# microsoft/UniVL

Measured on NVIDIA H100. Metric: video-text samples/sec, higher is better.
Workload: dtype bf16

## Files before the change

univl_b200/csrc/common.cuh:

```cuda
#pragma once

#include <cuda.h>
#include <cuda_bf16.h>
#include <cuda_runtime.h>
#include <stdint.h>
#include <stdio.h>

namespace univl {

typedef __nv_bfloat16 bf16;

int set_error(int code, const char* fmt, ...);
int device_sms();
int usable_sms();
int scratch_alloc(void** p, size_t bytes, cudaStream_t st);
int partials_reduce(float* part, int nparts, long long rows, long long cols, float* dst, long long ld, cudaStream_t st);
#define UNIVL_OK 0
#define UNIVL_ERR_ARG -1
#define UNIVL_ERR_CUDA -2
#define UNIVL_ERR_UNSUPPORTED -3

#define UNIVL_CHECK_ARG(cond, ...)                                   \
  do {                                                               \
    if (!(cond)) return univl::set_error(UNIVL_ERR_ARG, __VA_ARGS__); \
  } while (0)

#define UNIVL_CHECK_LAUNCH(name)                                                          \
  do {                                                                                    \
    cudaError_t e__ = cudaGetLastError();                                                 \
    if (e__ != cudaSuccess)                                                               \
      return univl::set_error(UNIVL_ERR_CUDA, "%s launch: %s", name, cudaGetErrorString(e__)); \
  } while (0)

bool pdl_enabled();
__device__ __forceinline__ void pdl_trigger() { asm volatile("griddepcontrol.launch_dependents;" ::: "memory"); }
__device__ __forceinline__ void pdl_wait() { asm volatile("griddepcontrol.wait;" ::: "memory"); }

template <typename... KArgs, typename... Args>
static inline cudaError_t launch_kernel(void (*kern)(KArgs...), dim3 grid, dim3 block, size_t smem, cudaStream_t st,
                                        Args... args) {
  cudaLaunchConfig_t cfg = {};
  cfg.gridDim = grid;
  cfg.blockDim = block;
  cfg.dynamicSmemBytes = smem;
  cfg.stream = st;
  cudaLaunchAttribute attr[1];
  int n = 0;
  if (pdl_enabled()) {
    attr[n].id = cudaLaunchAttributeProgrammaticStreamSerialization;
    attr[n].val.programmaticStreamSerializationAllowed = 1;
    ++n;
  }
  cfg.attrs = attr;
  cfg.numAttrs = n;
  return cudaLaunchKernelEx(&cfg, kern, KArgs(args)...);
}

__device__ __forceinline__ uint32_t smem_u32(const void* p) {
  return static_cast<uint32_t>(__cvta_generic_to_shared(p));
}
__device__ __forceinline__ uint32_t lane_id() { return threadIdx.x & 31u; }

__device__ __forceinline__ void pair_sources(long long p, int groups, long long n_seq, long long Nb, long long& i,
                                             long long& j) {
  if (groups == 0) {
    i = j = p;
    return;
  }
  const long long Gv = Nb / groups;
  const long long g = groups > 1 ? p / (n_seq / groups) : 0;
  const long long r = p - g * (n_seq / groups);
  i = g * (n_seq / Nb) + r / Gv;
  j = g * Gv + r % Gv;
}
__device__ __forceinline__ long long pair_sequence(int which, long long owner, int f, int groups, long long Gt,
                                                   long long Gv) {
  if (groups == 0) return owner;
  if (which == 0) return owner * Gv + f;
  const long long g = owner / Gv;
  return (g * Gt + f) * Gv + (owner - g * Gv);
}

__device__ __forceinline__ float warp_sum(float v) {
#pragma unroll
  for (int o = 16; o > 0; o >>= 1) v += __shfl_xor_sync(0xffffffffu, v, o);
  return v;
}
__device__ __forceinline__ float warp_max(float v) {
#pragma unroll
  for (int o = 16; o > 0; o >>= 1) v = fmaxf(v, __shfl_xor_sync(0xffffffffu, v, o));
  return v;
}

__device__ __forceinline__ uint32_t pack_bf16x2(float lo, float hi) {
  __nv_bfloat162 v = __floats2bfloat162_rn(lo, hi);
  return *reinterpret_cast<uint32_t*>(&v);
}
__device__ __forceinline__ float2 unpack_bf16x2(uint32_t u) {
  __nv_bfloat162 v = *reinterpret_cast<__nv_bfloat162*>(&u);
  return __bfloat1622float2(v);
}

__device__ __forceinline__ float rcp_approx(float x) {
  float r;
  asm("rcp.approx.ftz.f32 %0, %1;" : "=f"(r) : "f"(x));
  return r;
}
__device__ __forceinline__ float ex2_approx(float x) {
  float r;
  asm("ex2.approx.ftz.f32 %0, %1;" : "=f"(r) : "f"(x));
  return r;
}
__device__ __forceinline__ void erf_exp_terms(float x, float& w, float& gauss) {
  const float t = rcp_approx(fmaf(fabsf(x), 0.3275911f * 0.70710678118654752440f, 1.0f));
  gauss = ex2_approx((x * x) * (-0.5f * 1.44269504088896340736f));
  float poly = fmaf(0.5f * 1.061405429f, t, 0.5f * -1.453152027f);
  poly = fmaf(poly, t, 0.5f * 1.421413741f);
  poly = fmaf(poly, t, 0.5f * -0.284496736f);
  poly = fmaf(poly, t, 0.5f * 0.254829592f);
  w = (poly * t) * gauss;
}
__device__ __forceinline__ float gelu_erf(float x) {
  float w, g;
  erf_exp_terms(x, w, g);
  return fmaf(-fabsf(x), w, fmaxf(x, 0.f));
}
__device__ __forceinline__ float gelu_erf_grad(float x) {
  float w, g;
  erf_exp_terms(x, w, g);
  const float cdf = x >= 0.f ? 1.0f - w : w;
  return fmaf(x * 0.39894228040143267794f, g, cdf);
}

__device__ __forceinline__ uint4 philox4x32(uint64_t seed, uint64_t ctr_hi, uint64_t ctr_lo) {
  uint32_t k0 = (uint32_t)seed, k1 = (uint32_t)(seed >> 32);
  uint32_t c0 = (uint32_t)ctr_lo, c1 = (uint32_t)(ctr_lo >> 32);
  uint32_t c2 = (uint32_t)ctr_hi, c3 = (uint32_t)(ctr_hi >> 32);
#pragma unroll
  for (int i = 0; i < 10; ++i) {
    const uint32_t hi0 = __umulhi(0xD2511F53u, c0), lo0 = 0xD2511F53u * c0;
    const uint32_t hi1 = __umulhi(0xCD9E8D57u, c2), lo1 = 0xCD9E8D57u * c2;
    const uint32_t n0 = hi1 ^ c1 ^ k0, n1 = lo1, n2 = hi0 ^ c3 ^ k1, n3 = lo0;
    c0 = n0; c1 = n1; c2 = n2; c3 = n3;
    k0 += 0x9E3779B9u; k1 += 0xBB67AE85u;
  }
  return make_uint4(c0, c1, c2, c3);
}

__device__ __forceinline__ bool dropout_keep(uint64_t seed, uint64_t stream, uint64_t idx,
                                             uint32_t keep_threshold) {
  const uint4 r = philox4x32(seed, stream, idx >> 2);
  const uint32_t w = (idx & 3) == 0 ? r.x : (idx & 3) == 1 ? r.y : (idx & 3) == 2 ? r.z : r.w;
  return w < keep_threshold;
}
__host__ __device__ __forceinline__ uint32_t dropout_threshold(float p) {
  double keep = 1.0 - (double)p;
  if (keep >= 1.0) return 0xFFFFFFFFu;
  return (uint32_t)(keep * 4294967296.0);
}
__host__ __device__ __forceinline__ uint32_t dropout_threshold16(float p) {
  double keep = 1.0 - (double)p;
  if (keep >= 1.0) return 65536u;
  return (uint32_t)(keep * 65536.0 + 0.5);
}
__device__ __forceinline__ uint32_t philox_u16(const uint4& r, int w) {
  const uint32_t x = (w >> 1) == 0 ? r.x : (w >> 1) == 1 ? r.y : (w >> 1) == 2 ? r.z : r.w;
  return (w & 1) ? (x >> 16) : (x & 0xFFFFu);
}
__device__ __forceinline__ uint32_t dropout_keep8(uint64_t seed, uint64_t stream, uint64_t idx0, uint32_t thr16) {
  const uint4 r = philox4x32(seed, stream, idx0 >> 3);
  return ((r.x & 0xFFFFu) < thr16 ? 1u : 0u) | ((r.x >> 16) < thr16 ? 2u : 0u) | ((r.y & 0xFFFFu) < thr16 ? 4u : 0u) |
         ((r.y >> 16) < thr16 ? 8u : 0u) | ((r.z & 0xFFFFu) < thr16 ? 16u : 0u) | ((r.z >> 16) < thr16 ? 32u : 0u) |
         ((r.w & 0xFFFFu) < thr16 ? 64u : 0u) | ((r.w >> 16) < thr16 ? 128u : 0u);
}

__device__ __forceinline__ void mbar_init(uint64_t* bar, uint32_t count) {
  asm volatile("mbarrier.init.shared::cta.b64 [%0], %1;" ::"r"(smem_u32(bar)), "r"(count) : "memory");
}
__device__ __forceinline__ void fence_mbar_init() {
  asm volatile("fence.mbarrier_init.release.cluster;" ::: "memory");
}
__device__ __forceinline__ void fence_proxy_async_smem() {
  asm volatile("fence.proxy.async.shared::cta;" ::: "memory");
}
__device__ __forceinline__ void mbar_arrive_expect_tx(uint64_t* bar, uint32_t bytes) {
  asm volatile("mbarrier.arrive.expect_tx.shared::cta.b64 _, [%0], %1;" ::"r"(smem_u32(bar)), "r"(bytes)
               : "memory");
}
__device__ __forceinline__ void mbar_arrive(uint64_t* bar) {
  asm volatile("mbarrier.arrive.shared::cta.b64 _, [%0];" ::"r"(smem_u32(bar)) : "memory");
}
__device__ __forceinline__ uint32_t mbar_try_wait(uint64_t* bar, uint32_t parity) {
  uint32_t ok;
  asm volatile(
      "{\n\t.reg .pred p;\n\t"
      "mbarrier.try_wait.parity.shared::cta.b64 p, [%1], %2;\n\t"
      "selp.b32 %0, 1, 0, p;\n\t}"
      : "=r"(ok)
      : "r"(smem_u32(bar)), "r"(parity)
      : "memory");
  return ok;
}
__device__ __forceinline__ void mbar_wait(uint64_t* bar, uint32_t parity) {
  uint32_t spins = 0;
  while (!mbar_try_wait(bar, parity)) {
    if (++spins > (1u << 26)) __trap();
  }
}

__device__ __forceinline__ void tma_prefetch_desc(const CUtensorMap* m) {
  asm volatile("prefetch.tensormap [%0];" ::"l"(reinterpret_cast<uint64_t>(m)) : "memory");
}
__device__ __forceinline__ void tma_load_2d(void* smem_dst, const CUtensorMap* m, uint64_t* bar, int c0,
                                            int c1) {
  asm volatile(
      "cp.async.bulk.tensor.2d.shared::cluster.global.tile.mbarrier::complete_tx::bytes [%0], [%1, {%2, %3}], [%4];"
      ::"r"(smem_u32(smem_dst)), "l"(reinterpret_cast<uint64_t>(m)), "r"(c0), "r"(c1), "r"(smem_u32(bar))
      : "memory");
}


__device__ __forceinline__ void tma_store_2d(const CUtensorMap* m, const void* smem_src, int c0, int c1) {
  asm volatile("cp.async.bulk.tensor.2d.global.shared::cta.tile.bulk_group [%0, {%1, %2}], [%3];" ::"l"(
                   reinterpret_cast<uint64_t>(m)),
               "r"(c0), "r"(c1), "r"(smem_u32(smem_src))
               : "memory");
}
__device__ __forceinline__ void bulk_commit() { asm volatile("cp.async.bulk.commit_group;" ::: "memory"); }
template <int N>
__device__ __forceinline__ void bulk_wait_read() {
  asm volatile("cp.async.bulk.wait_group.read %0;" ::"n"(N) : "memory");
}
__device__ __forceinline__ void bulk_wait_all() { asm volatile("cp.async.bulk.wait_group 0;" ::: "memory"); }

__device__ __forceinline__ bool elect_one() {
  uint32_t pred;
  asm volatile(
      "{\n\t.reg .pred p;\n\t"
      "elect.sync _|p, 0xffffffff;\n\t"
      "selp.b32 %0, 1, 0, p;\n\t}"
      : "=r"(pred));
  return pred != 0;
}
__device__ __forceinline__ void wgmma_fence() { asm volatile("wgmma.fence.sync.aligned;" ::: "memory"); }
__device__ __forceinline__ void wgmma_commit() { asm volatile("wgmma.commit_group.sync.aligned;" ::: "memory"); }
template <int N>
__device__ __forceinline__ void wgmma_wait() {
  asm volatile("wgmma.wait_group.sync.aligned %0;" ::"n"(N) : "memory");
}
template <int R>
__device__ __forceinline__ void fence_regs(float (&d)[R]) {
#pragma unroll
  for (int i = 0; i < R; ++i) asm volatile("" : "+f"(d[i])::"memory");
}
template <int N>
__device__ __forceinline__ void regs_dealloc() {
  asm volatile("setmaxnreg.dec.sync.aligned.u32 %0;" ::"n"(N));
}
template <int N>
__device__ __forceinline__ void regs_alloc() {
  asm volatile("setmaxnreg.inc.sync.aligned.u32 %0;" ::"n"(N));
}
__device__ __forceinline__ void named_bar(int id, int count) {
  asm volatile("bar.sync %0, %1;" ::"r"(id), "r"(count) : "memory");
}

__device__ __forceinline__ uint64_t make_smem_desc_sw128(uint32_t smem_addr, uint32_t lbo_bytes, uint32_t sbo_bytes) {
  uint64_t d = 0;
  d |= (uint64_t)((smem_addr >> 4) & 0x3FFFu);
  d |= (uint64_t)((lbo_bytes >> 4) & 0x3FFFu) << 16;
  d |= (uint64_t)((sbo_bytes >> 4) & 0x3FFFu) << 32;
  d |= (uint64_t)1 << 62;
  return d;
}

}
```

univl_b200/csrc/gemm_wgmma.cu:

```cuda
#include "common.cuh"
#include "tmap.cuh"
#include "wgmma.cuh"

#include <stdio.h>

namespace univl {

enum GemmEpilogue : int {
  EPI_BIAS_BF16 = 0,
  EPI_BIAS_GELU_BF16 = 1,
  EPI_GELU_BWD_BF16 = 2,
  EPI_ADD_BF16 = 3,
  EPI_BIAS_F32 = 4,
  EPI_ATOMIC_F32 = 5,
};

struct GemmParams {
  int M, N, Kc;
  int k_blocks_per_split;
  int epilogue;
  float alpha;
  void* out;
  long long ldo;
  const float* bias;
  const bf16* aux_in;
  long long ld_aux_in;
  bf16* aux_out;
  long long ld_aux_out;
  int vec2;
  float* part;
};

constexpr int BLOCK_M = 128;
constexpr int BLOCK_K = 64;
constexpr int GEMM_THREADS = 384;
constexpr int PLAN_SMS = 132;

template <int BLOCK_N, int STAGES>
struct GemmSmem {
  static constexpr int A_BYTES = BLOCK_M * BLOCK_K * 2;
  static constexpr int B_BYTES = BLOCK_N * BLOCK_K * 2;
  static constexpr int STAGE_BYTES = A_BYTES + B_BYTES;
  static constexpr int BAR_OFFSET = STAGES * STAGE_BYTES;
  static constexpr int TOTAL = BAR_OFFSET + 2 * STAGES * 8;
  static constexpr int DYN_BYTES = TOTAL + 1024;
  static_assert(DYN_BYTES <= 227 * 1024, "shared memory per block");
};

struct WorkItem {
  int m0, n0, kb_begin, num_kb;
};
__device__ __forceinline__ WorkItem decode_work(int w, int m_tiles, int n_tiles, int total_kb, int kb_per, int bn) {
  const int tiles = m_tiles * n_tiles;
  const int split = w / tiles;
  const int rem = w - split * tiles;
  int m_blk, n_blk;
  if (kb_per >= total_kb) {
    m_blk = rem / n_tiles;
    n_blk = rem - m_blk * n_tiles;
  } else {
    n_blk = rem / m_tiles;
    m_blk = rem - n_blk * m_tiles;
  }
  WorkItem it;
  it.m0 = m_blk * BLOCK_M;
  it.n0 = n_blk * bn;
  it.kb_begin = split * kb_per;
  it.num_kb = min(total_kb, it.kb_begin + kb_per) - it.kb_begin;
  return it;
}

__device__ __forceinline__ void epi_pair(const GemmParams& p, int split, int row, int col, float v0, float v1) {
  if (row >= p.M || col >= p.N) return;
  const bool two = col + 1 < p.N;
  const bool vec = two && p.vec2;
  const int epi = p.epilogue;
  v0 *= p.alpha;
  v1 *= p.alpha;
  if (p.bias != nullptr && (epi == EPI_BIAS_BF16 || epi == EPI_BIAS_GELU_BF16 || epi == EPI_BIAS_F32)) {
    v0 += __ldg(p.bias + col);
    if (two) v1 += __ldg(p.bias + col + 1);
  }
  if (epi == EPI_ATOMIC_F32 && p.part != nullptr) {
    float* o = p.part + ((long long)split * p.M + row) * p.N + col;
    if (two && (p.N & 1) == 0) *reinterpret_cast<float2*>(o) = make_float2(v0, v1);
    else {
      o[0] = v0;
      if (two) o[1] = v1;
    }
    return;
  }
  if (epi == EPI_ATOMIC_F32 || epi == EPI_BIAS_F32) {
    float* o = reinterpret_cast<float*>(p.out) + (long long)row * p.ldo + col;
    if (epi == EPI_ATOMIC_F32) {
      if (vec) {
        float2 a = *reinterpret_cast<float2*>(o);
        *reinterpret_cast<float2*>(o) = make_float2(a.x + v0, a.y + v1);
      } else {
        o[0] += v0;
        if (two) o[1] += v1;
      }
    } else {
      if (vec) *reinterpret_cast<float2*>(o) = make_float2(v0, v1);
      else {
        o[0] = v0;
        if (two) o[1] = v1;
      }
    }
    return;
  }
  if (epi == EPI_GELU_BWD_BF16 || epi == EPI_ADD_BF16) {
    const bf16* a = p.aux_in + (long long)row * p.ld_aux_in + col;
    float x0, x1 = 0.f;
    if (vec) {
      const float2 f = unpack_bf16x2(*reinterpret_cast<const uint32_t*>(a));
      x0 = f.x;
      x1 = f.y;
    } else {
      x0 = __bfloat162float(a[0]);
      if (two) x1 = __bfloat162float(a[1]);
    }
    if (epi == EPI_GELU_BWD_BF16) {
      v0 *= gelu_erf_grad(x0);
      v1 *= gelu_erf_grad(x1);
    } else {
      v0 += x0;
      v1 += x1;
    }
  }
  if (epi == EPI_BIAS_GELU_BF16) {
    bf16* ao = p.aux_out + (long long)row * p.ld_aux_out + col;
    if (vec) *reinterpret_cast<uint32_t*>(ao) = pack_bf16x2(v0, v1);
    else {
      ao[0] = __float2bfloat16(v0);
      if (two) ao[1] = __float2bfloat16(v1);
    }
    v0 = gelu_erf(v0);
    v1 = gelu_erf(v1);
  }
  bf16* o = reinterpret_cast<bf16*>(p.out) + (long long)row * p.ldo + col;
  if (vec) *reinterpret_cast<uint32_t*>(o) = pack_bf16x2(v0, v1);
  else {
    o[0] = __float2bfloat16(v0);
    if (two) o[1] = __float2bfloat16(v1);
  }
}

constexpr int EPI_CHUNK = 8;

template <int EPI, bool BIAS, bool PART, int BLOCK_N>
__device__ __forceinline__ void epi_tile(const GemmParams& p, int split, int row, int col0,
                                         const float (&acc)[BLOCK_N / 2]) {
  constexpr int GROUPS = BLOCK_N / 8;
  constexpr int CHUNK = GROUPS < EPI_CHUNK ? GROUPS : EPI_CHUNK;
  constexpr bool AUX = EPI == EPI_GELU_BWD_BF16 || EPI == EPI_ADD_BF16;
  constexpr bool OUT_F32 = EPI == EPI_BIAS_F32 || EPI == EPI_ATOMIC_F32;
  constexpr bool ACCUM = EPI == EPI_ATOMIC_F32 && !PART;
  const float alpha = p.alpha;
  const float* bias = p.bias + col0;
  const bf16* ax = p.aux_in + (long long)row * p.ld_aux_in + col0;
  const long long ax8 = 8 * p.ld_aux_in;
  bf16* ao = p.aux_out + (long long)row * p.ld_aux_out + col0;
  const long long ao8 = 8 * p.ld_aux_out;
  const long long ld = PART ? (long long)p.N : p.ldo;
  const long long o8 = 8 * ld;
  float* of = PART ? p.part + ((long long)split * p.M + row) * p.N + col0
                   : reinterpret_cast<float*>(p.out) + (long long)row * ld + col0;
  bf16* ob = reinterpret_cast<bf16*>(p.out) + (long long)row * ld + col0;
  float b[2][CHUNK][2];
  uint32_t x[2][CHUNK][2];
  float2 a[2][CHUNK][2];
  auto load = [&](int j0, int s) {
#pragma unroll
    for (int j = 0; j < CHUNK; ++j) {
      const int c = (j0 + j) * 8;
      if constexpr (BIAS) {
        b[s][j][0] = __ldg(bias + c);
        b[s][j][1] = __ldg(bias + c + 1);
      }
#pragma unroll
      for (int h = 0; h < 2; ++h) {
        if constexpr (AUX) x[s][j][h] = *reinterpret_cast<const uint32_t*>(ax + h * ax8 + c);
        if constexpr (ACCUM) a[s][j][h] = *reinterpret_cast<const float2*>(of + h * o8 + c);
      }
    }
  };
  load(0, 0);
#pragma unroll
  for (int j0 = 0; j0 < GROUPS; j0 += CHUNK) {
    const int s = (j0 / CHUNK) & 1;
    if (j0 + CHUNK < GROUPS) load(j0 + CHUNK, s ^ 1);
#pragma unroll
    for (int j = 0; j < CHUNK; ++j) {
      const int c = (j0 + j) * 8;
#pragma unroll
      for (int h = 0; h < 2; ++h) {
        float v0 = __fmul_rn(acc[4 * (j0 + j) + 2 * h], alpha);
        float v1 = __fmul_rn(acc[4 * (j0 + j) + 2 * h + 1], alpha);
        if constexpr (BIAS) {
          v0 = __fadd_rn(v0, b[s][j][0]);
          v1 = __fadd_rn(v1, b[s][j][1]);
        }
        if constexpr (AUX) {
          const float2 f = unpack_bf16x2(x[s][j][h]);
          if constexpr (EPI == EPI_GELU_BWD_BF16) {
            v0 = __fmul_rn(v0, gelu_erf_grad(f.x));
            v1 = __fmul_rn(v1, gelu_erf_grad(f.y));
          } else {
            v0 = __fadd_rn(v0, f.x);
            v1 = __fadd_rn(v1, f.y);
          }
        }
        if constexpr (OUT_F32) {
          if constexpr (ACCUM) {
            v0 = __fadd_rn(a[s][j][h].x, v0);
            v1 = __fadd_rn(a[s][j][h].y, v1);
          }
          *reinterpret_cast<float2*>(of + h * o8 + c) = make_float2(v0, v1);
        } else {
          if constexpr (EPI == EPI_BIAS_GELU_BF16) {
            *reinterpret_cast<uint32_t*>(ao + h * ao8 + c) = pack_bf16x2(v0, v1);
            v0 = gelu_erf(v0);
            v1 = gelu_erf(v1);
          }
          *reinterpret_cast<uint32_t*>(ob + h * o8 + c) = pack_bf16x2(v0, v1);
        }
      }
    }
  }
}

template <int BLOCK_N, int STAGES, bool A_MN, bool B_MN>
__global__ void __launch_bounds__(GEMM_THREADS, 1)
gemm_wgmma_kernel(const __grid_constant__ CUtensorMap tmap_a, const __grid_constant__ CUtensorMap tmap_b,
                  const GemmParams p, const int num_work) {
  using L = GemmSmem<BLOCK_N, STAGES>;
  pdl_trigger();
  extern __shared__ uint8_t smem_raw[];
  uint8_t* smem = reinterpret_cast<uint8_t*>((reinterpret_cast<uintptr_t>(smem_raw) + 1023) & ~uintptr_t(1023));
  uint64_t* full_bar = reinterpret_cast<uint64_t*>(smem + L::BAR_OFFSET);
  uint64_t* empty_bar = full_bar + STAGES;

  const int wg = threadIdx.x >> 7;
  const int m_tiles = (p.M + BLOCK_M - 1) / BLOCK_M;
  const int n_tiles = (p.N + BLOCK_N - 1) / BLOCK_N;
  const int total_kb = (p.Kc + BLOCK_K - 1) / BLOCK_K;
  const int kb_per = p.k_blocks_per_split;

  if (threadIdx.x == 0) {
    tma_prefetch_desc(&tmap_a);
    tma_prefetch_desc(&tmap_b);
    for (int s = 0; s < STAGES; ++s) {
      mbar_init(&full_bar[s], 1);
      mbar_init(&empty_bar[s], 2);
    }
    fence_mbar_init();
  }
  __syncthreads();
  pdl_wait();

  if (wg == 0) {
    regs_dealloc<40>();
    if (threadIdx.x == 0) {
      uint32_t it = 0;
      for (int w = blockIdx.x; w < num_work; w += gridDim.x) {
        const WorkItem wi = decode_work(w, m_tiles, n_tiles, total_kb, kb_per, BLOCK_N);
        for (int i = 0; i < wi.num_kb; ++i, ++it) {
          const int s = it % STAGES;
          const uint32_t ph = (it / STAGES) & 1;
          mbar_wait(&empty_bar[s], ph ^ 1);
          uint8_t* sa = smem + s * L::STAGE_BYTES;
          uint8_t* sb = sa + L::A_BYTES;
          mbar_arrive_expect_tx(&full_bar[s], L::STAGE_BYTES);
          const int k_elem = (wi.kb_begin + i) * BLOCK_K;
          if (!A_MN) {
            tma_load_2d(sa, &tmap_a, &full_bar[s], k_elem, wi.m0);
          } else {
#pragma unroll
            for (int c = 0; c < BLOCK_M / 64; ++c)
              tma_load_2d(sa + c * (BLOCK_K * 128), &tmap_a, &full_bar[s], wi.m0 + c * 64, k_elem);
          }
          if (!B_MN) {
            tma_load_2d(sb, &tmap_b, &full_bar[s], k_elem, wi.n0);
          } else {
#pragma unroll
            for (int c = 0; c < BLOCK_N / 64; ++c)
              tma_load_2d(sb + c * (BLOCK_K * 128), &tmap_b, &full_bar[s], wi.n0 + c * 64, k_elem);
          }
        }
      }
    }
  } else {
    regs_alloc<232>();
    const int c = wg - 1;
    const int t = threadIdx.x & 127;
    const int warp = t >> 5, lane = t & 31;
    uint32_t it = 0;
    for (int w = blockIdx.x; w < num_work; w += gridDim.x) {
      const WorkItem wi = decode_work(w, m_tiles, n_tiles, total_kb, kb_per, BLOCK_N);
      float acc[BLOCK_N / 2];
#pragma unroll
      for (int e = 0; e < BLOCK_N / 2; ++e) acc[e] = 0.f;
      int prev_s = -1;
      for (int i = 0; i < wi.num_kb; ++i, ++it) {
        const int s = it % STAGES;
        const uint32_t ph = (it / STAGES) & 1;
        mbar_wait(&full_bar[s], ph);
        const uint32_t sa = smem_u32(smem + s * L::STAGE_BYTES) + c * (64 * 128);
        const uint32_t sb = smem_u32(smem + s * L::STAGE_BYTES) + L::A_BYTES;
        wgmma_fence();
        fence_regs(acc);
#pragma unroll
        for (int k = 0; k < BLOCK_K / 16; ++k) {
          const uint64_t da = A_MN ? make_smem_desc_sw128(sa + k * 2048, BLOCK_K * 128, 1024)
                                   : make_smem_desc_sw128(sa + k * 32, 16, 1024);
          const uint64_t db = B_MN ? make_smem_desc_sw128(sb + k * 2048, BLOCK_K * 128, 1024)
                                   : make_smem_desc_sw128(sb + k * 32, 16, 1024);
          WgmmaSS<BLOCK_N>::template mma<A_MN ? 1 : 0, B_MN ? 1 : 0>(acc, da, db, (i > 0 || k > 0) ? 1 : 0);
        }
        wgmma_commit();
        fence_regs(acc);
        wgmma_wait<1>();
        if (prev_s >= 0 && t == 0) mbar_arrive(&empty_bar[prev_s]);
        prev_s = s;
      }
      wgmma_wait<0>();
      fence_regs(acc);
      if (t == 0) mbar_arrive(&empty_bar[prev_s]);
      const int row = wi.m0 + c * 64 + warp * 16 + (lane >> 2);
      const int col0 = wi.n0 + 2 * (lane & 3);
      const int split = wi.kb_begin / kb_per;
      const bool inside = p.vec2 && wi.m0 + BLOCK_M <= p.M && wi.n0 + BLOCK_N <= p.N &&
                          (p.part == nullptr || (p.N & 1) == 0);
      if (inside) {
        const bool bias = p.bias != nullptr;
        switch (p.epilogue) {
          case EPI_BIAS_BF16:
            if (bias) epi_tile<EPI_BIAS_BF16, true, false, BLOCK_N>(p, split, row, col0, acc);
            else epi_tile<EPI_BIAS_BF16, false, false, BLOCK_N>(p, split, row, col0, acc);
            break;
          case EPI_BIAS_GELU_BF16:
            if (bias) epi_tile<EPI_BIAS_GELU_BF16, true, false, BLOCK_N>(p, split, row, col0, acc);
            else epi_tile<EPI_BIAS_GELU_BF16, false, false, BLOCK_N>(p, split, row, col0, acc);
            break;
          case EPI_GELU_BWD_BF16:
            epi_tile<EPI_GELU_BWD_BF16, false, false, BLOCK_N>(p, split, row, col0, acc);
            break;
          case EPI_ADD_BF16:
            epi_tile<EPI_ADD_BF16, false, false, BLOCK_N>(p, split, row, col0, acc);
            break;
          case EPI_BIAS_F32:
            if (bias) epi_tile<EPI_BIAS_F32, true, false, BLOCK_N>(p, split, row, col0, acc);
            else epi_tile<EPI_BIAS_F32, false, false, BLOCK_N>(p, split, row, col0, acc);
            break;
          default:
            if (p.part != nullptr) epi_tile<EPI_ATOMIC_F32, false, true, BLOCK_N>(p, split, row, col0, acc);
            else epi_tile<EPI_ATOMIC_F32, false, false, BLOCK_N>(p, split, row, col0, acc);
        }
      } else {
#pragma unroll
        for (int j = 0; j < BLOCK_N / 8; ++j) {
          if (wi.n0 + j * 8 >= p.N) break;
          epi_pair(p, split, row, col0 + j * 8, acc[4 * j], acc[4 * j + 1]);
          epi_pair(p, split, row + 8, col0 + j * 8, acc[4 * j + 2], acc[4 * j + 3]);
        }
      }
    }
  }
}

template <int BLOCK_N, int STAGES, bool A_MN, bool B_MN>
static int launch_gemm(const CUtensorMap& ta, const CUtensorMap& tb, const GemmParams& p, int splits,
                       cudaStream_t stream) {
  using L = GemmSmem<BLOCK_N, STAGES>;
  auto kern = gemm_wgmma_kernel<BLOCK_N, STAGES, A_MN, B_MN>;
  cudaError_t e = cudaFuncSetAttribute(kern, cudaFuncAttributeMaxDynamicSharedMemorySize, L::DYN_BYTES);
  if (e != cudaSuccess) return set_error(UNIVL_ERR_CUDA, "gemm smem attribute: %s", cudaGetErrorString(e));
  const int sms = usable_sms();
  const long long work =
      (long long)((p.M + BLOCK_M - 1) / BLOCK_M) * ((p.N + BLOCK_N - 1) / BLOCK_N) * (long long)splits;
  if (work > 0x7fffffffLL) return set_error(UNIVL_ERR_ARG, "gemm: too many tiles");
  const int grid = (int)(work < sms ? work : sms);
  e = launch_kernel(kern, dim3(grid), dim3(GEMM_THREADS), (size_t)L::DYN_BYTES, stream, ta, tb, p, (int)work);
  if (e != cudaSuccess) return set_error(UNIVL_ERR_CUDA, "gemm launch: %s", cudaGetErrorString(e));
  UNIVL_CHECK_LAUNCH("gemm_wgmma");
  return UNIVL_OK;
}

template <int BLOCK_N, int STAGES>
static int dispatch_major(bool a_mn, bool b_mn, const CUtensorMap& ta, const CUtensorMap& tb, const GemmParams& p,
                          int splits, cudaStream_t stream) {
  if (!a_mn && !b_mn) return launch_gemm<BLOCK_N, STAGES, false, false>(ta, tb, p, splits, stream);
  if (!a_mn && b_mn) return launch_gemm<BLOCK_N, STAGES, false, true>(ta, tb, p, splits, stream);
  if (a_mn && b_mn) return launch_gemm<BLOCK_N, STAGES, true, true>(ta, tb, p, splits, stream);
  return launch_gemm<BLOCK_N, STAGES, true, false>(ta, tb, p, splits, stream);
}

}

using namespace univl;

namespace {
struct GemmPlan {
  int bn, splits, kb_per;
};
int plan_gemm(int M, int N, int Kc, int epilogue, int block_n, int split_k, GemmPlan* plan) {
  const int total_kb = (Kc + BLOCK_K - 1) / BLOCK_K;
  const int m_tiles = (M + BLOCK_M - 1) / BLOCK_M;
  int bn = block_n;
  if (bn == 0) {
    bn = 256;
    if (epilogue != EPI_ATOMIC_F32)
      while (bn > 64 && (long long)m_tiles * ((N + bn - 1) / bn) < PLAN_SMS) bn >>= 1;
    if (N <= 64) bn = 64;
    else if (N <= 128 && bn > 128) bn = 128;
  }
  UNIVL_CHECK_ARG(bn == 64 || bn == 128 || bn == 256, "gemm: block_n must be 64/128/256");
  const int n_tiles = (N + bn - 1) / bn;
  int splits = 1;
  if (epilogue == EPI_ATOMIC_F32) {
    splits = split_k;
    if (splits == 0) {
      const long long tiles = (long long)m_tiles * n_tiles;
      splits = (int)((2 * PLAN_SMS + tiles - 1) / tiles);
      if (splits > total_kb / 2) splits = total_kb / 2;
      if (splits < 1) splits = 1;
    }
    if (splits > total_kb) splits = total_kb;
  }
  const int kb_per = (total_kb + splits - 1) / splits;
  splits = (total_kb + kb_per - 1) / kb_per;
  plan->bn = bn; plan->splits = splits; plan->kb_per = kb_per;
  return UNIVL_OK;
}
}

extern "C" int univl_gemm_plan(int M, int N, int Kc, int epilogue, int block_n, int split_k) {
  GemmPlan plan;
  if (int rc = plan_gemm(M, N, Kc, epilogue, block_n, split_k, &plan)) return rc;
  return 1;
}

extern "C" int univl_gemm_bf16(const void* A, long long lda, int a_mn_major, const void* B, long long ldb,
                               int b_mn_major, int M, int N, int Kc, void* out, long long ldo, int epilogue,
                               const float* bias, const void* aux_in, long long ld_aux_in, void* aux_out,
                               long long ld_aux_out, float alpha, int block_n, int split_k, void* stream_) {
  cudaStream_t stream = reinterpret_cast<cudaStream_t>(stream_);
  UNIVL_CHECK_ARG(M > 0 && N > 0 && Kc > 0, "gemm: empty problem M=%d N=%d K=%d", M, N, Kc);
  UNIVL_CHECK_ARG(A && B && out, "gemm: null operand");
  UNIVL_CHECK_ARG((lda % 8) == 0 && (ldb % 8) == 0, "gemm: lda/ldb must be multiples of 8 elements (got %lld, %lld)",
                  lda, ldb);
  UNIVL_CHECK_ARG(((uintptr_t)A & 15) == 0 && ((uintptr_t)B & 15) == 0, "gemm: operands must be 16-byte aligned");
  UNIVL_CHECK_ARG(epilogue >= 0 && epilogue <= 5, "gemm: unknown epilogue %d", epilogue);
  if (epilogue == EPI_GELU_BWD_BF16 || epilogue == EPI_ADD_BF16)
    UNIVL_CHECK_ARG(aux_in != nullptr, "gemm: epilogue %d needs aux_in", epilogue);
  if (epilogue == EPI_BIAS_GELU_BF16) UNIVL_CHECK_ARG(aux_out != nullptr, "gemm: gelu epilogue needs aux_out");
  UNIVL_CHECK_ARG(split_k >= 0, "gemm: bad split_k");
  if (epilogue != EPI_ATOMIC_F32) UNIVL_CHECK_ARG(split_k <= 1, "gemm: split_k>1 needs the atomic epilogue");

  GemmPlan plan;
  if (int prc = plan_gemm(M, N, Kc, epilogue, block_n, split_k, &plan)) return prc;
  const int bn = plan.bn;

  CUtensorMap ta, tb;
  int rc;
  if (!a_mn_major) rc = make_tmap(&ta, A, M, Kc, lda, BLOCK_M);
  else             rc = make_tmap(&ta, A, Kc, M, lda, BLOCK_K);
  if (rc) return rc;
  if (!b_mn_major) rc = make_tmap(&tb, B, N, Kc, ldb, bn);
  else             rc = make_tmap(&tb, B, Kc, N, ldb, BLOCK_K);
  if (rc) return rc;

  GemmParams p;
  p.M = M; p.N = N; p.Kc = Kc;
  p.k_blocks_per_split = plan.kb_per;
  p.epilogue = epilogue;
  p.alpha = alpha;
  p.out = out; p.ldo = ldo;
  p.bias = bias;
  p.aux_in = reinterpret_cast<const bf16*>(aux_in); p.ld_aux_in = ld_aux_in;
  p.aux_out = reinterpret_cast<bf16*>(aux_out); p.ld_aux_out = ld_aux_out;
  const bool out_f32 = epilogue == EPI_BIAS_F32 || epilogue == EPI_ATOMIC_F32;
  bool vec2 = ((uintptr_t)out % (out_f32 ? 8 : 4)) == 0 && (ldo % 2) == 0;
  if (aux_in != nullptr) vec2 = vec2 && ((uintptr_t)aux_in % 4) == 0 && (ld_aux_in % 2) == 0;
  if (aux_out != nullptr) vec2 = vec2 && ((uintptr_t)aux_out % 4) == 0 && (ld_aux_out % 2) == 0;
  p.vec2 = vec2 ? 1 : 0;
  p.part = nullptr;
  if (plan.splits > 1)
    if ((rc = scratch_alloc((void**)&p.part, (size_t)plan.splits * M * N * sizeof(float), stream))) return rc;

  const bool amn = a_mn_major != 0, bmn = b_mn_major != 0;
  if (bn == 256) rc = dispatch_major<256, 4>(amn, bmn, ta, tb, p, plan.splits, stream);
  else if (bn == 128) rc = dispatch_major<128, 6>(amn, bmn, ta, tb, p, plan.splits, stream);
  else rc = dispatch_major<64, 8>(amn, bmn, ta, tb, p, plan.splits, stream);
  if (rc != UNIVL_OK || p.part == nullptr) return rc;
  return partials_reduce(p.part, plan.splits, M, N, reinterpret_cast<float*>(out), ldo, stream);
}
```

Baseline: 1181.

## Ping-pong consumer warpgroups over whole tiles and widen bf16 epilogue stores

For block widths up to 128, each consumer warpgroup now computes a full 128-row tile on alternating work items. Named barriers hand the tensor cores from one group to the other, so one group's epilogue overlaps the other's MMAs. The bf16 epilogue gains a 16-byte store path that regroups fragments across a lane quad with shuffles, and the planner picks 128-wide tiles more often. The risks are extra register pressure from two accumulator sets per warpgroup and shuffle overhead in the epilogue.

```diff
diff --git a/univl_b200/csrc/common.cuh b/univl_b200/csrc/common.cuh
--- a/univl_b200/csrc/common.cuh
+++ b/univl_b200/csrc/common.cuh
@@ -264,6 +264,9 @@
 __device__ __forceinline__ void named_bar(int id, int count) {
   asm volatile("bar.sync %0, %1;" ::"r"(id), "r"(count) : "memory");
 }
+__device__ __forceinline__ void named_bar_arrive(int id, int count) {
+  asm volatile("bar.arrive %0, %1;" ::"r"(id), "r"(count) : "memory");
+}
 
 __device__ __forceinline__ uint64_t make_smem_desc_sw128(uint32_t smem_addr, uint32_t lbo_bytes, uint32_t sbo_bytes) {
   uint64_t d = 0;
diff --git a/univl_b200/csrc/gemm_wgmma.cu b/univl_b200/csrc/gemm_wgmma.cu
--- a/univl_b200/csrc/gemm_wgmma.cu
+++ b/univl_b200/csrc/gemm_wgmma.cu
@@ -28,6 +28,7 @@
   bf16* aux_out;
   long long ld_aux_out;
   int vec2;
+  int vec8;
   float* part;
 };
 
@@ -148,15 +149,42 @@
 
 constexpr int EPI_CHUNK = 8;
 
-template <int EPI, bool BIAS, bool PART, int BLOCK_N>
+__device__ __forceinline__ uint4 quad_transpose(uint32_t w0, uint32_t w1, uint32_t w2, uint32_t w3, int q) {
+  const bool odd = q & 1;
+  uint32_t r0 = __shfl_xor_sync(0xffffffffu, odd ? w0 : w1, 1);
+  uint32_t r1 = __shfl_xor_sync(0xffffffffu, odd ? w2 : w3, 1);
+  if (odd) {
+    w0 = r0;
+    w2 = r1;
+  } else {
+    w1 = r0;
+    w3 = r1;
+  }
+  const bool hi = q & 2;
+  r0 = __shfl_xor_sync(0xffffffffu, hi ? w0 : w2, 2);
+  r1 = __shfl_xor_sync(0xffffffffu, hi ? w1 : w3, 2);
+  if (hi) {
+    w0 = r0;
+    w1 = r1;
+  } else {
+    w2 = r0;
+    w3 = r1;
+  }
+  return make_uint4(w0, w1, w2, w3);
+}
+
+template <int EPI, bool BIAS, bool PART, int BLOCK_N, bool WIDE = false>
 __device__ __forceinline__ void epi_tile(const GemmParams& p, int split, int row, int col0,
                                          const float (&acc)[BLOCK_N / 2]) {
   constexpr int GROUPS = BLOCK_N / 8;
-  constexpr int CHUNK = GROUPS < EPI_CHUNK ? GROUPS : EPI_CHUNK;
+  constexpr int CHUNK = WIDE ? 4 : (GROUPS < EPI_CHUNK ? GROUPS : EPI_CHUNK);
+  static_assert(CHUNK % 4 == 0, "a chunk holds whole quads of 8-column groups");
   constexpr bool AUX = EPI == EPI_GELU_BWD_BF16 || EPI == EPI_ADD_BF16;
   constexpr bool OUT_F32 = EPI == EPI_BIAS_F32 || EPI == EPI_ATOMIC_F32;
+  static_assert(!(WIDE && OUT_F32), "16-byte stores are for the bf16 outputs");
   constexpr bool ACCUM = EPI == EPI_ATOMIC_F32 && !PART;
   const float alpha = p.alpha;
+  const int q = threadIdx.x & 3;
   const float* bias = p.bias + col0;
   const bf16* ax = p.aux_in + (long long)row * p.ld_aux_in + col0;
   const long long ax8 = 8 * p.ld_aux_in;
@@ -191,50 +219,123 @@
     const int s = (j0 / CHUNK) & 1;
     if (j0 + CHUNK < GROUPS) load(j0 + CHUNK, s ^ 1);
 #pragma unroll
-    for (int j = 0; j < CHUNK; ++j) {
-      const int c = (j0 + j) * 8;
+    for (int jq = 0; jq < CHUNK; jq += 4) {
 #pragma unroll
       for (int h = 0; h < 2; ++h) {
-        float v0 = __fmul_rn(acc[4 * (j0 + j) + 2 * h], alpha);
-        float v1 = __fmul_rn(acc[4 * (j0 + j) + 2 * h + 1], alpha);
-        if constexpr (BIAS) {
-          v0 = __fadd_rn(v0, b[s][j][0]);
-          v1 = __fadd_rn(v1, b[s][j][1]);
-        }
-        if constexpr (AUX) {
-          const float2 f = unpack_bf16x2(x[s][j][h]);
-          if constexpr (EPI == EPI_GELU_BWD_BF16) {
-            v0 = __fmul_rn(v0, gelu_erf_grad(f.x));
-            v1 = __fmul_rn(v1, gelu_erf_grad(f.y));
+        uint32_t wo[4], wa[4];
+#pragma unroll
+        for (int jj = 0; jj < 4; ++jj) {
+          const int j = jq + jj;
+          const int c = (j0 + j) * 8;
+          float v0 = __fmul_rn(acc[4 * (j0 + j) + 2 * h], alpha);
+          float v1 = __fmul_rn(acc[4 * (j0 + j) + 2 * h + 1], alpha);
+          if constexpr (BIAS) {
+            v0 = __fadd_rn(v0, b[s][j][0]);
+            v1 = __fadd_rn(v1, b[s][j][1]);
+          }
+          if constexpr (AUX) {
+            const float2 f = unpack_bf16x2(x[s][j][h]);
+            if constexpr (EPI == EPI_GELU_BWD_BF16) {
+              v0 = __fmul_rn(v0, gelu_erf_grad(f.x));
+              v1 = __fmul_rn(v1, gelu_erf_grad(f.y));
+            } else {
+              v0 = __fadd_rn(v0, f.x);
+              v1 = __fadd_rn(v1, f.y);
+            }
+          }
+          if constexpr (OUT_F32) {
+            if constexpr (ACCUM) {
+              v0 = __fadd_rn(a[s][j][h].x, v0);
+              v1 = __fadd_rn(a[s][j][h].y, v1);
+            }
+            *reinterpret_cast<float2*>(of + h * o8 + c) = make_float2(v0, v1);
           } else {
-            v0 = __fadd_rn(v0, f.x);
-            v1 = __fadd_rn(v1, f.y);
+            if constexpr (EPI == EPI_BIAS_GELU_BF16) {
+              const uint32_t w = pack_bf16x2(v0, v1);
+              if constexpr (WIDE) wa[jj] = w;
+              else *reinterpret_cast<uint32_t*>(ao + h * ao8 + c) = w;
+              v0 = gelu_erf(v0);
+              v1 = gelu_erf(v1);
+            }
+            const uint32_t w = pack_bf16x2(v0, v1);
+            if constexpr (WIDE) wo[jj] = w;
+            else *reinterpret_cast<uint32_t*>(ob + h * o8 + c) = w;
           }
         }
-        if constexpr (OUT_F32) {
-          if constexpr (ACCUM) {
-            v0 = __fadd_rn(a[s][j][h].x, v0);
-            v1 = __fadd_rn(a[s][j][h].y, v1);
-          }
-          *reinterpret_cast<float2*>(of + h * o8 + c) = make_float2(v0, v1);
+        if constexpr (WIDE) {
+          const int c = (j0 + jq) * 8 + 6 * q;
+          if constexpr (EPI == EPI_BIAS_GELU_BF16)
+            *reinterpret_cast<uint4*>(ao + h * ao8 + c) = quad_transpose(wa[0], wa[1], wa[2], wa[3], q);
+          *reinterpret_cast<uint4*>(ob + h * o8 + c) = quad_transpose(wo[0], wo[1], wo[2], wo[3], q);
+        }
+      }
+    }
+  }
+}
+
+template <int BLOCK_N>
+__device__ __forceinline__ void epilogue_block(const GemmParams& p, bool inside, int split, int n0, int row, int col0,
+                                               const float (&acc)[BLOCK_N / 2]) {
+  if (inside) {
+    const bool bias = p.bias != nullptr;
+    const bool wide = p.vec8;
+    switch (p.epilogue) {
+      case EPI_BIAS_BF16:
+        if (wide) {
+          if (bias) epi_tile<EPI_BIAS_BF16, true, false, BLOCK_N, true>(p, split, row, col0, acc);
+          else epi_tile<EPI_BIAS_BF16, false, false, BLOCK_N, true>(p, split, row, col0, acc);
         } else {
-          if constexpr (EPI == EPI_BIAS_GELU_BF16) {
-            *reinterpret_cast<uint32_t*>(ao + h * ao8 + c) = pack_bf16x2(v0, v1);
-            v0 = gelu_erf(v0);
-            v1 = gelu_erf(v1);
-          }
-          *reinterpret_cast<uint32_t*>(ob + h * o8 + c) = pack_bf16x2(v0, v1);
+          if (bias) epi_tile<EPI_BIAS_BF16, true, false, BLOCK_N>(p, split, row, col0, acc);
+          else epi_tile<EPI_BIAS_BF16, false, false, BLOCK_N>(p, split, row, col0, acc);
         }
-      }
-    }
-  }
-}
+        break;
+      case EPI_BIAS_GELU_BF16:
+        if (wide) {
+          if (bias) epi_tile<EPI_BIAS_GELU_BF16, true, false, BLOCK_N, true>(p, split, row, col0, acc);
+          else epi_tile<EPI_BIAS_GELU_BF16, false, false, BLOCK_N, true>(p, split, row, col0, acc);
+        } else {
+          if (bias) epi_tile<EPI_BIAS_GELU_BF16, true, false, BLOCK_N>(p, split, row, col0, acc);
+          else epi_tile<EPI_BIAS_GELU_BF16, false, false, BLOCK_N>(p, split, row, col0, acc);
+        }
+        break;
+      case EPI_GELU_BWD_BF16:
+        if (wide) epi_tile<EPI_GELU_BWD_BF16, false, false, BLOCK_N, true>(p, split, row, col0, acc);
+        else epi_tile<EPI_GELU_BWD_BF16, false, false, BLOCK_N>(p, split, row, col0, acc);
+        break;
+      case EPI_ADD_BF16:
+        if (wide) epi_tile<EPI_ADD_BF16, false, false, BLOCK_N, true>(p, split, row, col0, acc);
+        else epi_tile<EPI_ADD_BF16, false, false, BLOCK_N>(p, split, row, col0, acc);
+        break;
+      case EPI_BIAS_F32:
+        if (bias) epi_tile<EPI_BIAS_F32, true, false, BLOCK_N>(p, split, row, col0, acc);
+        else epi_tile<EPI_BIAS_F32, false, false, BLOCK_N>(p, split, row, col0, acc);
+        break;
+      default:
+        if (p.part != nullptr) epi_tile<EPI_ATOMIC_F32, false, true, BLOCK_N>(p, split, row, col0, acc);
+        else epi_tile<EPI_ATOMIC_F32, false, false, BLOCK_N>(p, split, row, col0, acc);
+    }
+  } else {
+#pragma unroll
+    for (int j = 0; j < BLOCK_N / 8; ++j) {
+      if (n0 + j * 8 >= p.N) break;
+      epi_pair(p, split, row, col0 + j * 8, acc[4 * j], acc[4 * j + 1]);
+      epi_pair(p, split, row + 8, col0 + j * 8, acc[4 * j + 2], acc[4 * j + 3]);
+    }
+  }
+}
+
+__device__ __forceinline__ bool tile_inside(const GemmParams& p, const WorkItem& wi, int bn) {
+  return p.vec2 && wi.m0 + BLOCK_M <= p.M && wi.n0 + bn <= p.N && (p.part == nullptr || (p.N & 1) == 0);
+}
+
+constexpr int TURN_BAR = 1;
 
 template <int BLOCK_N, int STAGES, bool A_MN, bool B_MN>
 __global__ void __launch_bounds__(GEMM_THREADS, 1)
 gemm_wgmma_kernel(const __grid_constant__ CUtensorMap tmap_a, const __grid_constant__ CUtensorMap tmap_b,
                   const GemmParams p, const int num_work) {
   using L = GemmSmem<BLOCK_N, STAGES>;
+  constexpr bool PING = BLOCK_N <= 128;
   pdl_trigger();
   extern __shared__ uint8_t smem_raw[];
   uint8_t* smem = reinterpret_cast<uint8_t*>((reinterpret_cast<uintptr_t>(smem_raw) + 1023) & ~uintptr_t(1023));
@@ -252,7 +353,7 @@
     tma_prefetch_desc(&tmap_b);
     for (int s = 0; s < STAGES; ++s) {
       mbar_init(&full_bar[s], 1);
-      mbar_init(&empty_bar[s], 2);
+      mbar_init(&empty_bar[s], PING ? 1 : 2);
     }
     fence_mbar_init();
   }
@@ -290,7 +391,7 @@
         }
       }
     }
-  } else {
+  } else if constexpr (!PING) {
     regs_alloc<232>();
     const int c = wg - 1;
     const int t = threadIdx.x & 127;
@@ -329,42 +430,65 @@
       if (t == 0) mbar_arrive(&empty_bar[prev_s]);
       const int row = wi.m0 + c * 64 + warp * 16 + (lane >> 2);
       const int col0 = wi.n0 + 2 * (lane & 3);
+      epilogue_block<BLOCK_N>(p, tile_inside(p, wi, BLOCK_N), wi.kb_begin / kb_per, wi.n0, row, col0, acc);
+    }
+  } else {
+    regs_alloc<232>();
+    const int c = wg - 1;
+    const int t = threadIdx.x & 127;
+    const int warp = t >> 5, lane = t & 31;
+    uint32_t it = 0;
+    int j = 0;
+    for (int w = blockIdx.x; w < num_work; w += gridDim.x, ++j) {
+      const WorkItem wi = decode_work(w, m_tiles, n_tiles, total_kb, kb_per, BLOCK_N);
+      if ((j & 1) != c) {
+        it += wi.num_kb;
+        continue;
+      }
+      float acc[2][BLOCK_N / 2];
+#pragma unroll
+      for (int e = 0; e < BLOCK_N / 2; ++e) acc[0][e] = acc[1][e] = 0.f;
+      if (j > 0) named_bar(TURN_BAR + c, 256);
+      int prev_s = -1;
+      for (int i = 0; i < wi.num_kb; ++i, ++it) {
+        const int s = it % STAGES;
+        const uint32_t ph = (it / STAGES) & 1;
+        mbar_wait(&full_bar[s], ph);
+        const uint32_t sa = smem_u32(smem + s * L::STAGE_BYTES);
+        const uint32_t sb = sa + L::A_BYTES;
+        wgmma_fence();
+        fence_regs(acc[0]);
+        fence_regs(acc[1]);
+#pragma unroll
+        for (int k = 0; k < BLOCK_K / 16; ++k) {
+          const uint64_t db = B_MN ? make_smem_desc_sw128(sb + k * 2048, BLOCK_K * 128, 1024)
+                                   : make_smem_desc_sw128(sb + k * 32, 16, 1024);
+#pragma unroll
+          for (int h = 0; h < 2; ++h) {
+            const uint32_t sah = sa + h * (64 * 128);
+            const uint64_t da = A_MN ? make_smem_desc_sw128(sah + k * 2048, BLOCK_K * 128, 1024)
+                                     : make_smem_desc_sw128(sah + k * 32, 16, 1024);
+            WgmmaSS<BLOCK_N>::template mma<A_MN ? 1 : 0, B_MN ? 1 : 0>(acc[h], da, db, (i > 0 || k > 0) ? 1 : 0);
+          }
+        }
+        wgmma_commit();
+        fence_regs(acc[0]);
+        fence_regs(acc[1]);
+        wgmma_wait<1>();
+        if (prev_s >= 0 && t == 0) mbar_arrive(&empty_bar[prev_s]);
+        prev_s = s;
+      }
+      if (w + (int)gridDim.x < num_work) named_bar_arrive(TURN_BAR + (c ^ 1), 256);
+      wgmma_wait<0>();
+      fence_regs(acc[0]);
+      fence_regs(acc[1]);
+      if (t == 0) mbar_arrive(&empty_bar[prev_s]);
+      const bool inside = tile_inside(p, wi, BLOCK_N);
       const int split = wi.kb_begin / kb_per;
-      const bool inside = p.vec2 && wi.m0 + BLOCK_M <= p.M && wi.n0 + BLOCK_N <= p.N &&
-                          (p.part == nullptr || (p.N & 1) == 0);
-      if (inside) {
-        const bool bias = p.bias != nullptr;
-        switch (p.epilogue) {
-          case EPI_BIAS_BF16:
-            if (bias) epi_tile<EPI_BIAS_BF16, true, false, BLOCK_N>(p, split, row, col0, acc);
-            else epi_tile<EPI_BIAS_BF16, false, false, BLOCK_N>(p, split, row, col0, acc);
-            break;
-          case EPI_BIAS_GELU_BF16:
-            if (bias) epi_tile<EPI_BIAS_GELU_BF16, true, false, BLOCK_N>(p, split, row, col0, acc);
-            else epi_tile<EPI_BIAS_GELU_BF16, false, false, BLOCK_N>(p, split, row, col0, acc);
-            break;
-          case EPI_GELU_BWD_BF16:
-            epi_tile<EPI_GELU_BWD_BF16, false, false, BLOCK_N>(p, split, row, col0, acc);
-            break;
-          case EPI_ADD_BF16:
-            epi_tile<EPI_ADD_BF16, false, false, BLOCK_N>(p, split, row, col0, acc);
-            break;
-          case EPI_BIAS_F32:
-            if (bias) epi_tile<EPI_BIAS_F32, true, false, BLOCK_N>(p, split, row, col0, acc);
-            else epi_tile<EPI_BIAS_F32, false, false, BLOCK_N>(p, split, row, col0, acc);
-            break;
-          default:
-            if (p.part != nullptr) epi_tile<EPI_ATOMIC_F32, false, true, BLOCK_N>(p, split, row, col0, acc);
-            else epi_tile<EPI_ATOMIC_F32, false, false, BLOCK_N>(p, split, row, col0, acc);
-        }
-      } else {
-#pragma unroll
-        for (int j = 0; j < BLOCK_N / 8; ++j) {
-          if (wi.n0 + j * 8 >= p.N) break;
-          epi_pair(p, split, row, col0 + j * 8, acc[4 * j], acc[4 * j + 1]);
-          epi_pair(p, split, row + 8, col0 + j * 8, acc[4 * j + 2], acc[4 * j + 3]);
-        }
-      }
+      const int row = wi.m0 + warp * 16 + (lane >> 2);
+      const int col0 = wi.n0 + 2 * (lane & 3);
+      epilogue_block<BLOCK_N>(p, inside, split, wi.n0, row, col0, acc[0]);
+      epilogue_block<BLOCK_N>(p, inside, split, wi.n0, row + 64, col0, acc[1]);
     }
   }
 }
@@ -410,8 +534,11 @@
   int bn = block_n;
   if (bn == 0) {
     bn = 256;
-    if (epilogue != EPI_ATOMIC_F32)
-      while (bn > 64 && (long long)m_tiles * ((N + bn - 1) / bn) < PLAN_SMS) bn >>= 1;
+    if (epilogue != EPI_ATOMIC_F32) {
+      const auto tiles = [&](int w) { return (long long)m_tiles * ((N + w - 1) / w); };
+      if (tiles(256) < 2 * PLAN_SMS) bn = 128;
+      if (tiles(128) < PLAN_SMS) bn = 64;
+    }
     if (N <= 64) bn = 64;
     else if (N <= 128 && bn > 128) bn = 128;
   }
@@ -485,6 +612,9 @@
   if (aux_in != nullptr) vec2 = vec2 && ((uintptr_t)aux_in % 4) == 0 && (ld_aux_in % 2) == 0;
   if (aux_out != nullptr) vec2 = vec2 && ((uintptr_t)aux_out % 4) == 0 && (ld_aux_out % 2) == 0;
   p.vec2 = vec2 ? 1 : 0;
+  bool vec8 = !out_f32 && ((uintptr_t)out % 16) == 0 && (ldo % 8) == 0;
+  if (aux_out != nullptr) vec8 = vec8 && ((uintptr_t)aux_out % 16) == 0 && (ld_aux_out % 8) == 0;
+  p.vec8 = vec8 ? 1 : 0;
   p.part = nullptr;
   if (plan.splits > 1)
     if ((rc = scratch_alloc((void**)&p.part, (size_t)plan.splits * M * N * sizeof(float), stream))) return rc;
```

Result: faster. 1298, median of 6 (+9.9%).
